# juanmc2005/diart

Measured on NVIDIA H100. Metric: audio-seconds/sec (real-time factor) at 5s/0.5s step, batch 256, higher is better.
Workload: dtype f32

## Files before the change

### diart_b200/csrc/api_seg.cu

```cuda
#include <math.h>
#include <string.h>

#include <algorithm>
#include <memory>
#include <vector>

#include "host.cuh"

namespace dg {

static void sinc_filters(const float* low_hz_, const float* band_hz_, std::vector<float>& filt ) {
  filt.assign(251 * 80, 0.f);
  float n_[125], win[125];
  for (int i = 0; i < 125; i++) {
    const float t = (float)(i - 125) / 16000.0f;
    n_[i] = 6.283185307179586f * t;
    win[i] = (float)(0.54 - 0.46 * cos(2.0 * M_PI * i / 250.0));
  }
  for (int f = 0; f < 40; f++) {
    const float low = 50.f + fabsf(low_hz_[f]);
    float high = low + 50.f + fabsf(band_hz_[f]);
    high = fminf(fmaxf(high, 50.f), 8000.f);
    const float band = high - low, two_band = 2.f * band;
    for (int i = 0; i < 125; i++) {
// ... 276 lines not shown
  h->K = (int)cn;
  const float* cw = t.get("classifier.weight", cn * 128);
  const float* cb = t.get("classifier.bias", cn);
  if (!cw || !cb) return DG_EWEIGHT;
  if (upload(h->cw, std::vector<float>(cw, cw + cn * 128)) || upload(h->cb, std::vector<float>(cb, cb + cn)))
    return DG_ECUDA;
  return 0;
}

extern "C" int dg_seg_create(const dg_tensor* tensors, int n, int device, dg_seg** out) {
  if (!tensors || !out) {
    set_error("dg_seg_create: null argument");
    return DG_EINVAL;
  }
  DG_CUDA(cudaSetDevice(device));
  std::unique_ptr<dg_seg> h(new dg_seg());
  h->device = device;
  Tensors t(tensors, n);
  int rc = seg_prepare(h.get(), t);
  if (rc) return rc;
  *out = h.release();
  return DG_OK;
}

extern "C" int dg_seg_dims(const dg_seg* h, int num_samples, int* frames, int* speakers) {
  if (!h || num_samples < 3000) {
    set_error("dg_seg_dims: bad arguments");
    return DG_EINVAL;
  }
  Geom g = make_geom(num_samples);
  if (frames) *frames = g.T2;
  if (speakers) *speakers = h->ps_speakers ? h->ps_speakers : h->K;
  return DG_OK;
}

extern "C" int dg_seg_set_powerset(dg_seg* h, int num_speakers, int max_per_frame) {
  if (!h || num_speakers < 1 || num_speakers > 8 || max_per_frame < 0 || max_per_frame > num_speakers) {
    set_error("dg_seg_set_powerset: bad arguments");
    return DG_EINVAL;
  }
  std::vector<uint32_t> masks;
  for (int size = 0; size <= max_per_frame; size++)
    for (uint32_t m = 0; m < (1u << num_speakers); m++) {
      if (__builtin_popcount(m) != size) continue;
      masks.push_back(m);
    }
  auto members = [&](uint32_t m) {
    std::vector<int> v;
    for (int i = 0; i < num_speakers; i++)
      if (m >> i & 1u) v.push_back(i);
    return v;
  };
  std::stable_sort(masks.begin(), masks.end(), [&](uint32_t a, uint32_t b) {
    const int sa = __builtin_popcount(a), sb = __builtin_popcount(b);
    if (sa != sb) return sa < sb;
    return members(a) < members(b);
  });
  if ((int)masks.size() != h->K) {
    set_error("dg_seg_set_powerset: the classifier has " + std::to_string(h->K) + " outputs but the powerset has " +
              std::to_string(masks.size()) + " classes");
    return DG_EINVAL;
  }
  DG_CUDA(cudaSetDevice(h->device));
  if (h->ps_masks.ensure(masks.size() * 4)) return DG_ECUDA;
  DG_CUDA(cudaMemcpy(h->ps_masks.p, masks.data(), masks.size() * 4, cudaMemcpyHostToDevice));
  h->ps_speakers = num_speakers;
  return DG_OK;
}

static int seg_head_final(dg_seg* h, const float* y2, int B, const Geom& g, float* seg, cudaStream_t st) {
  if (h->ps_speakers)
    return launch_seg_powerset(y2, h->cw.as<float>(), h->cb.as<float>(), B, g.T2, g.S2, h->K, h->ps_speakers,
                               h->ps_masks.as<unsigned>(), seg, st);
  return launch_seg_final(y2, h->cw.as<float>(), h->cb.as<float>(), B, g.T2, g.S2, h->K, seg, st);
}

int seg_forward_lane(dg_seg* h, int lane, const SincPrep* prep, const float* wav, int B, int S, float* seg,
                     cudaStream_t st, int stop_after) {
  DG_CUDA(cudaSetDevice(h->device));
  dg_seg::Scratch& w = h->scr[lane];
  const Geom g = make_geom(S);
  int rc;
  if ((rc = run_sincnet(h->sw, w.work, wav, B, g, st, prep))) return rc;
  const size_t rows = (size_t)B * g.S2 + 64;
  if (w.gx.ensure(rows * 1024 * 4) || w.y2.ensure(rows * 128 * 4) || w.xh.ensure(rows * 256 * 2) ||
      w.xl.ensure(rows * 256 * 2) || w.y1h.ensure(rows * 128 * 2) || w.y1l.ensure(rows * 128 * 2))
    return DG_ECUDA;
  const long long M = (long long)B * g.S2;
  if ((rc = launch_split_ex(w.work.out, M, 64, 64, 64, w.work.out_pool, g.S2, w.work.sc2.as<float>(), w.work.sh2.as<float>(),
                            w.xh.p, w.xl.p, st)))
    return rc;
  for (int L = 0; L < 4 && L <= stop_after; L++) {
    const int cin = L == 0 ? 64 : 256;
    TcGemm t{};
    t.A_hi = w.xh.p; t.A_lo = w.xl.p; t.lda = cin; t.Cin = cin; t.KW = 1; t.dil = 1; t.Mtot = M; t.M = M;
    t.N = 1024; t.bias = h->bih[L].as<float>(); t.out_f32 = w.gx.as<float>(); t.ldc = 1024; t.epi = 0; t.tag = "lstm_inproj";
    if ((rc = set_weights(t, h->wih[L])) || (rc = launch_gemm_tc(t, st))) return rc;
    if ((rc = launch_lstm_layer_tc(w.gx.as<float>(), h->whh[L].hi.p, h->whh[L].lo.p, h->whh[L].scale, B, g.T2, g.S2, nullptr,
                                   w.xh.p, w.xl.p, st)))
      return rc;
  }
  if (stop_after < 3) return 0;
  TcGemm t{};
  t.A_hi = w.xh.p; t.A_lo = w.xl.p; t.lda = 256; t.Cin = 256; t.KW = 1; t.dil = 1; t.Mtot = M; t.M = M;
  t.N = 128; t.bias = h->l1b.as<float>(); t.bn_scale = h->ones128.as<float>(); t.bn_shift = h->zeros128.as<float>();
  t.out_hi = w.y1h.p; t.out_lo = w.y1l.p; t.ldc = 128; t.epi = 1; t.tag = "seg_linear";
  if ((rc = set_weights(t, h->l1)) || (rc = launch_gemm_tc(t, st))) return rc;
  t.A_hi = w.y1h.p; t.A_lo = w.y1l.p; t.lda = 128; t.Cin = 128; t.bias = h->l2b.as<float>();
  t.out_hi = nullptr; t.out_lo = nullptr; t.out_f32 = w.y2.as<float>(); t.epi = 2;
  if ((rc = set_weights(t, h->l2)) || (rc = launch_gemm_tc(t, st))) return rc;
  return seg_head_final(h, w.y2.as<float>(), B, g, seg, st);
}

extern "C" int dg_seg_forward(dg_seg* h, const float* wav, int B, int S, float* seg, void* stream) {
  if (!h || !wav || !seg || B < 1 || S < 3000) {
    set_error("dg_seg_forward: bad arguments (need B >= 1, S >= 3000)");
    return DG_EINVAL;
  }
  cudaStream_t st = (cudaStream_t)stream;
  DG_CUDA(cudaSetDevice(h->device));
  LaneUse use(h->guard[0], stream ? stream : (void*)h, st);
  int rc;
  if ((rc = use.rc) || (rc = seg_forward_lane(h, 0, nullptr, wav, B, S, seg, st))) return rc;
  return use.end();
}

extern "C" int dg_seg_debug_stage(dg_seg* h, const float* wav_dev, int B, int S, int hop, int stage, float* out_host, int64_t cap,
                                  int* dims) {
  if (!h || !wav_dev || !out_host || !dims || B < 1 || S < 3000 || hop < 0 || stage < 0 || stage > 10 || h->ps_speakers) {
    set_error("dg_seg_debug_stage: bad arguments (need a multilabel segmentation handle, B >= 1, S >= 3000, stage 0..10)");
    return DG_EINVAL;
  }
  DG_CUDA(cudaSetDevice(h->device));
  const Geom g = make_geom(S);
  const char* who = "dg_seg_debug_stage";
  cudaStream_t st = nullptr;
  SincPrep shared;
  const SincPrep* prep = nullptr;
  DevBuf seg;
  int rc;
  if (seg.ensure((size_t)B * g.T2 * h->K * 4)) return DG_ECUDA;
  {
    LaneUse use(h->guard[0], h, st);
    if ((rc = use.rc)) return rc;
    if (hop > 0) {
      if ((rc = run_sinc_prep(shared, wav_dev, B, g, st, hop, false))) return rc;
      prep = &shared;
    }
    if ((rc = seg_forward_lane(h, 0, prep, wav_dev, B, S, seg.as<float>(), st, stage <= 3 ? -1 : stage <= 7 ? stage - 4 : 99)))
      return rc;
  }
  DG_CUDA(cudaDeviceSynchronize());
  if ((rc = debug_front_paths(prep, g, &dims[3]))) return rc;
  if (lstm_tc_rows(B) == 16) dims[3] |= DG_DBG_LSTM_16ROWS;
  const dg_seg::Scratch& w = h->scr[0];
  if (stage <= 3) return debug_copy_front(who, stage, w.work, prep, w.xh.p, w.xl.p, B, g, out_host, cap, dims);
  if (stage <= 7) return debug_copy_map(who, w.xh.p, w.xl.p, B, g.S2, 256, g.T2, 256, out_host, cap, dims);
  if (stage == 8) return debug_copy_map(who, w.y1h.p, w.y1l.p, B, g.S2, 128, g.T2, 128, out_host, cap, dims);
  if (stage == 9) return debug_copy_map(who, w.y2.p, nullptr, B, g.S2, 128, g.T2, 128, out_host, cap, dims);
  return debug_copy_map(who, seg.p, nullptr, B, g.T2, h->K, g.T2, h->K, out_host, cap, dims);
}

extern "C" int dg_seg_destroy(dg_seg* h) {
  delete h;
  return DG_OK;
}
```

### diart_b200/csrc/lstm_tc.cu

```cuda
#include <stdio.h>
#include <stdlib.h>
#include <string.h>

#include <vector>

#include "dg_common.cuh"
#include "tc_ptx.cuh"

namespace dg {

constexpr int LT_THREADS = 512;
constexpr int LT_WS_BYTES = 2 * 512 * 128;
__host__ __device__ constexpr int lt_plane(int nb) { return 128 * nb * 2; }
__host__ __device__ constexpr int lt_h_bytes(int nb) { return 2 * 2 * lt_plane(nb); }
__host__ __device__ constexpr int lt_x_bytes(int nb) { return 512 * nb * 4; }
constexpr int lt_smem(int nb) { return LT_WS_BYTES + lt_h_bytes(nb) + 2 * lt_x_bytes(nb) + 64 + 1024; }
static_assert(lt_smem(16) <= 227 * 1024, "lstm_tc: shared memory over the per-block limit");
static int lt_rows(int B) { return B >= 128 ? 16 : 8; }

__device__ __forceinline__ float ex2_approx(float x) {
  float y;
  asm("ex2.approx.ftz.f32 %0, %1;" : "=f"(y) : "f"(x));
  return y;
}
__device__ __forceinline__ float rcp_approx(float x) {
  float y;
  asm("rcp.approx.ftz.f32 %0, %1;" : "=f"(y) : "f"(x));
  return y;
}

__host__ __device__ constexpr int lt_row(int g, int u) { return (u >> 5) * 128 + (g >> 1) * 64 + ((u & 31) >> 3) * 16 + (g & 1) * 8 + (u & 7); }

template <int NB>
__global__ void __launch_bounds__(LT_THREADS, 1)
lstm_tc_kernel(const __grid_constant__ CUtensorMap tm_wlo, const __grid_constant__ CUtensorMap tm_gx,
               const uint16_t* __restrict__ w_hi , int B, int T, int stride, int groups_per_dir,
               float* __restrict__ hout, uint16_t* __restrict__ out_hi, uint16_t* __restrict__ out_lo, float acc_scale) {
  constexpr int LT_PLANE = lt_plane(NB), LT_H_BYTES = lt_h_bytes(NB), LT_X_BYTES = lt_x_bytes(NB);
  constexpr int E = NB / 4;
  extern __shared__ unsigned char smem_raw[];
  unsigned char* smem = reinterpret_cast<unsigned char*>((reinterpret_cast<uintptr_t>(smem_raw) + 1023) & ~uintptr_t(1023));
  unsigned char* wsm = smem;
  unsigned char* hsm = smem + LT_WS_BYTES;
  unsigned char* xsm = hsm + LT_H_BYTES;
  uint64_t* w_full = reinterpret_cast<uint64_t*>(xsm + 2 * LT_X_BYTES);
  uint64_t* x_full = w_full + 1;
  const int warp = threadIdx.x >> 5, lane = threadIdx.x & 31;
  const int wg = warp >> 2, wq = warp & 3;
  const int dir = blockIdx.x / groups_per_dir;
  const int b0 = (blockIdx.x - dir * groups_per_dir) * NB;
  const int t0 = dir == 0 ? 0 : T - 1;
  const int dt = dir == 0 ? 1 : -1;

  if (threadIdx.x == 0) {
    mbar_init(w_full, 1);
    mbar_init(&x_full[0], 1);
    mbar_init(&x_full[1], 1);
    asm volatile("fence.mbarrier_init.release.cluster;" ::: "memory");
  }
  for (int i = threadIdx.x; i < LT_H_BYTES / 4; i += LT_THREADS) reinterpret_cast<uint32_t*>(hsm)[i] = 0u;
  __syncthreads();
  if (threadIdx.x == 0) {
    mbar_expect_tx(w_full, LT_WS_BYTES);
    for (int kb = 0; kb < 2; kb++)
      for (int half = 0; half < 2; half++)
        tma_load_2d(wsm + kb * 65536 + half * 32768, &tm_wlo, kb * 64, dir * 512 + half * 256, w_full);
    mbar_expect_tx(&x_full[0], LT_X_BYTES);
    tma_load_4d(xsm, &tm_gx, 0, b0, dir * 16, t0, &x_full[0]);
  }
  uint32_t wa[2][8][4];
  {
    const uint32_t* src = reinterpret_cast<const uint32_t*>(w_hi + (size_t)dir * 512 * 128);
#pragma unroll
    for (int t = 0; t < 2; t++) {
      const int r0 = wg * 128 + t * 64 + wq * 16 + (lane >> 2);
#pragma unroll
      for (int ks = 0; ks < 8; ks++) {
        const int k2 = (ks * 16 + 2 * (lane & 3)) >> 1;
        wa[t][ks][0] = src[(size_t)r0 * 64 + k2];
        wa[t][ks][1] = src[(size_t)(r0 + 8) * 64 + k2];
        wa[t][ks][2] = src[(size_t)r0 * 64 + k2 + 4];
        wa[t][ks][3] = src[(size_t)(r0 + 8) * 64 + k2 + 4];
      }
    }
  }
  asm volatile("fence.proxy.async.shared::cta;" ::: "memory");
  __syncthreads();
  mbar_wait(w_full, 0);

  const int u = wg * 32 + wq * 8 + (lane >> 2);
  const int n0 = 2 * (lane & 3);
  auto ne = [](int e) { return (e & 1) + 8 * (e >> 1); };
  bool valid[E];
#pragma unroll
  for (int e = 0; e < E; e++) valid[e] = b0 + n0 + ne(e) < B;
  int hrow = (b0 + n0) * stride + t0;
  uint32_t x_addr[2];
#pragma unroll
  for (int j = 0; j < 2; j++) x_addr[j] = smem_u32(xsm) + wg * NB * 128 + (n0 + j) * 128 + ((((u & 31) >> 2) ^ (n0 + j)) << 4) + (u & 3) * 4;
  const uint32_t h_addr = smem_u32(hsm) + (u >> 3) * NB * 16 + n0 * 16 + (u & 7) * 2;
  const uint32_t wlo0 = smem_u32(wsm) + (wg * 128) * 128;
  const float L2E = 1.4426950408889634f;
  float c[E] = {};
  for (int step = 0; step < T; step++) {
    const int buf = step & 1;
    const uint32_t hb = smem_u32(hsm) + buf * (LT_H_BYTES / 2);
    uint32_t wlo = wlo0;
    asm volatile("" : "+r"(wlo));
    float acc[2][NB / 2];
    wg_fence();
#pragma unroll
    for (int ks = 0; ks < 8; ks++) {
      const uint64_t bh = wg_desc_plain(hb + ks * NB * 32, NB * 16, 128),
                     bl = wg_desc_plain(hb + LT_PLANE + ks * NB * 32, NB * 16, 128);
#pragma unroll
      for (int t = 0; t < 2; t++) {
        const uint64_t al = wg_desc(wlo + (ks >> 2) * 65536 + t * 64 * 128) + (uint64_t)(((ks & 3) * 32) >> 4);
        wgmma_rs<NB>(acc[t], wa[t][ks], bl, ks != 0);
        wgmma_ss<NB>(acc[t], al, bh, 1);
        wgmma_rs<NB>(acc[t], wa[t][ks], bh, 1);
      }
    }
    wg_commit();
    if (threadIdx.x == 0 && step + 1 < T) {
      uint64_t* bar = &x_full[(step + 1) & 1];
      mbar_expect_tx(bar, LT_X_BYTES);
      tma_load_4d(xsm + ((step + 1) & 1) * LT_X_BYTES, &tm_gx, 0, b0, dir * 16, t0 + (step + 1) * dt, bar);
    }
    wg_wait<0>();
    wg_fence_acc(acc[0]);
    wg_fence_acc(acc[1]);
    mbar_wait(&x_full[buf], (step >> 1) & 1);
    float h[E];
    uint16_t hh[E], hl[E];
#pragma unroll
    for (int e = 0; e < E; e++) {
      const int a = 4 * (e >> 1) + (e & 1);
      const uint32_t xa = x_addr[e & 1] + buf * LT_X_BYTES + (e >> 1) * 1024;
      float xg[4];
#pragma unroll
      for (int g = 0; g < 4; g++) asm volatile("ld.shared.f32 %0, [%1];" : "=f"(xg[g]) : "r"(xa + g * 4 * NB * 128) : "memory");
      const float di = 1.f + ex2_approx(fminf(fmaf(acc[0][a], acc_scale, xg[0]) * -L2E, 40.f));
      const float df = 1.f + ex2_approx(fminf(fmaf(acc[0][a + 2], acc_scale, xg[1]) * -L2E, 40.f));
      const float eg = ex2_approx(fminf(fmaf(acc[1][a], acc_scale, xg[2]) * (2.f * L2E), 40.f));
      const float p = di * (1.f + eg);
      c[e] = fmaf(c[e], p, (eg - 1.f) * df) * rcp_approx(p * df);
      const float ec = ex2_approx(fminf(c[e] * (2.f * L2E), 40.f));
      const float eo = ex2_approx(fminf(fmaf(acc[1][a + 2], acc_scale, xg[3]) * -L2E, 40.f));
      h[e] = valid[e] ? (ec - 1.f) * rcp_approx((1.f + eo) * (ec + 1.f)) : 0.f;
      split_h16(h[e], hh[e], hl[e]);
    }
    const uint32_t dst = h_addr + (buf ^ 1) * (LT_H_BYTES / 2);
#pragma unroll
    for (int e = 0; e < E; e++) {
      const uint32_t o = (e & 1) * 16 + (e >> 1) * 128;
      asm volatile("st.shared.u16 [%0], %1;" ::"r"(dst + o), "h"(hh[e]) : "memory");
      asm volatile("st.shared.u16 [%0], %1;" ::"r"(dst + LT_PLANE + o), "h"(hl[e]) : "memory");
    }
    asm volatile("fence.proxy.async.shared::cta;" ::: "memory");
    __syncthreads();
#pragma unroll
    for (int e = 0; e < E; e++)
      if (valid[e]) {
        const size_t o = (size_t)(hrow + ne(e) * stride) * 256 + dir * 128 + u;
        if (out_hi) {
          out_hi[o] = hh[e];
          out_lo[o] = hl[e];
        }
        if (hout) hout[o] = h[e];
      }
    hrow += dt;
  }
}

size_t lstm_tc_plane_elems() { return (size_t)2 * 512 * 128; }

float lstm_tc_pack_whh(const float* whh_fwd, const float* whh_bwd, uint16_t* hi, uint16_t* lo) {
  const float s0 = weight_plane_scale(whh_fwd, 512 * 128), s1 = weight_plane_scale(whh_bwd, 512 * 128);
  const float scale = s0 < s1 ? s0 : s1;
  std::vector<float> perm((size_t)512 * 128);
  for (int d = 0; d < 2; d++) {
    const float* w = d == 0 ? whh_fwd : whh_bwd;
    for (int g = 0; g < 4; g++)
      for (int u = 0; u < 128; u++) memcpy(&perm[(size_t)lt_row(g, u) * 128], w + ((size_t)g * 128 + u) * 128, 128 * sizeof(float));
    split_weights_host(perm.data(), 512, 512, 128, hi + (size_t)d * 512 * 128, lo + (size_t)d * 512 * 128, scale);
  }
  return scale;
}

int launch_lstm_layer_tc(const float* gx, const void* whh_hi, const void* whh_lo, float w_scale, int B, int T, int stride,
                         float* hout, void* out_hi, void* out_lo, cudaStream_t st) {
  ProfScope _ps("lstm_rec", st);
  EncodeTiledFn fn = encode_fn();
  if (!fn) {
    set_error("cuTensorMapEncodeTiled is not available from the driver");
    return -2;
  }
  if (!hout && !out_hi) {
    set_error("lstm_rec: no output buffer");
    return -1;
  }
  CUtensorMap tm;
  cuuint64_t dims[2] = {128, 1024};
  cuuint64_t strides[1] = {256};
  cuuint32_t box[2] = {64, 256};
  cuuint32_t estr[2] = {1, 1};
  if (fn(&tm, CU_TENSOR_MAP_DATA_TYPE_BFLOAT16, 2, const_cast<void*>(whh_lo), dims, strides, box, estr,
         CU_TENSOR_MAP_INTERLEAVE_NONE, CU_TENSOR_MAP_SWIZZLE_128B, CU_TENSOR_MAP_L2_PROMOTION_L2_256B,
         CU_TENSOR_MAP_FLOAT_OOB_FILL_NONE) != CUDA_SUCCESS) {
    set_error("cuTensorMapEncodeTiled failed for W_hh");
    return -2;
  }
  const int nb = lt_rows(B);
  CUtensorMap tmx;
  cuuint64_t xdims[4] = {32, (cuuint64_t)B, 32, (cuuint64_t)T};
  cuuint64_t xstrides[3] = {(cuuint64_t)stride * 4096, 128, 4096};
  cuuint32_t xbox[4] = {32, (cuuint32_t)nb, 16, 1};
  cuuint32_t xestr[4] = {1, 1, 1, 1};
  if (fn(&tmx, CU_TENSOR_MAP_DATA_TYPE_FLOAT32, 4, const_cast<float*>(gx), xdims, xstrides, xbox, xestr,
         CU_TENSOR_MAP_INTERLEAVE_NONE, CU_TENSOR_MAP_SWIZZLE_128B, CU_TENSOR_MAP_L2_PROMOTION_L2_256B,
         CU_TENSOR_MAP_FLOAT_OOB_FILL_NONE) != CUDA_SUCCESS) {
    set_error("cuTensorMapEncodeTiled failed for the LSTM gate rows");
    return -2;
  }
  auto kern = nb == 16 ? lstm_tc_kernel<16> : lstm_tc_kernel<8>;
  const int smem = lt_smem(nb);
  static bool attr_done[2][64] = {};
  if (first_use_on_device(attr_done[nb == 16])) DG_CUDA(cudaFuncSetAttribute(kern, cudaFuncAttributeMaxDynamicSharedMemorySize, smem));
  const int gpd = (B + nb - 1) / nb;
  const float inv = w_scale > 0.f ? 1.f / w_scale : 1.f;
  kern<<<2 * gpd, LT_THREADS, smem, st>>>(tm, tmx, reinterpret_cast<const uint16_t*>(whh_hi), B, T, stride, gpd, hout,
                                          reinterpret_cast<uint16_t*>(out_hi), reinterpret_cast<uint16_t*>(out_lo), inv);
  DG_LAUNCHED();
  return 0;
}

int lstm_tc_rows(int B) { return lt_rows(B); }
int lstm_tc_ctas(int B) { return 2 * ((B + lt_rows(B) - 1) / lt_rows(B)); }

}
```

### diart_b200/csrc/tc_ptx.cuh

```cuda
#pragma once
#include <cuda.h>
#include <cuda_bf16.h>
#include <stdint.h>

#include "dg_common.cuh"

namespace dg {

__device__ __forceinline__ uint32_t smem_u32(const void* p) { return (uint32_t)__cvta_generic_to_shared(p); }

__device__ __forceinline__ void mbar_init(uint64_t* bar, uint32_t count) {
  asm volatile("mbarrier.init.shared::cta.b64 [%0], %1;" ::"r"(smem_u32(bar)), "r"(count));
}
__device__ __forceinline__ void mbar_expect_tx(uint64_t* bar, uint32_t bytes) {
  asm volatile("mbarrier.arrive.expect_tx.shared::cta.b64 _, [%0], %1;" ::"r"(smem_u32(bar)), "r"(bytes) : "memory");
}
__device__ __forceinline__ void mbar_arrive(uint64_t* bar) {
  asm volatile("mbarrier.arrive.shared::cta.b64 _, [%0];" ::"r"(smem_u32(bar)) : "memory");
}
__device__ __forceinline__ bool mbar_try_wait(uint64_t* bar, uint32_t parity) {
  uint32_t ok;
  asm volatile(
      "{\n.reg .pred p;\nmbarrier.try_wait.parity.shared::cta.b64 p, [%1], %2;\nselp.u32 %0, 1, 0, p;\n}"
      : "=r"(ok)
      : "r"(smem_u32(bar)), "r"(parity)
      : "memory");
  return ok != 0;
}
__device__ __forceinline__ bool mbar_test_wait(uint64_t* bar, uint32_t parity) {
  uint32_t ok;
  asm volatile(
      "{\n.reg .pred p;\nmbarrier.test_wait.parity.shared::cta.b64 p, [%1], %2;\nselp.u32 %0, 1, 0, p;\n}"
      : "=r"(ok)
      : "r"(smem_u32(bar)), "r"(parity)
      : "memory");
  return ok != 0;
}
__device__ __forceinline__ void mbar_wait(uint64_t* bar, uint32_t parity) {
  if (mbar_try_wait(bar, parity)) return;
  const long long t0 = clock64();
  while (!mbar_try_wait(bar, parity)) {
    if (clock64() - t0 > 4000000000LL) __trap();
  }
}
__device__ __forceinline__ void tma_load_2d(void* smem_dst, const CUtensorMap* tmap, int c0, int c1, uint64_t* bar) {
  asm volatile(
      "cp.async.bulk.tensor.2d.shared::cluster.global.tile.mbarrier::complete_tx::bytes [%0], [%1, {%2, %3}], [%4];"
      ::"r"(smem_u32(smem_dst)), "l"(reinterpret_cast<uint64_t>(tmap)), "r"(c0), "r"(c1), "r"(smem_u32(bar))
      : "memory");
}
__device__ __forceinline__ void tma_load_4d(void* smem_dst, const CUtensorMap* tmap, int c0, int c1, int c2, int c3,
                                            uint64_t* bar) {
  asm volatile(
      "cp.async.bulk.tensor.4d.shared::cluster.global.tile.mbarrier::complete_tx::bytes [%0], [%1, {%2, %3, %4, %5}], [%6];"
      ::"r"(smem_u32(smem_dst)), "l"(reinterpret_cast<uint64_t>(tmap)), "r"(c0), "r"(c1), "r"(c2), "r"(c3), "r"(smem_u32(bar))
      : "memory");
}

__device__ __forceinline__ uint16_t f32_to_h16(float x) {
  uint16_t r;
  asm("cvt.rn.satfinite.f16.f32 %0, %1;" : "=h"(r) : "f"(x));
  return r;
}
__device__ __forceinline__ float h16_to_f32(uint16_t h) {
  float f;
  asm("cvt.f32.f16 %0, %1;" : "=f"(f) : "h"(h));
  return f;
}
__device__ __forceinline__ void split_h16(float x, uint16_t& hi, uint16_t& lo) {
  hi = f32_to_h16(x);
  lo = f32_to_h16(x - h16_to_f32(hi));
}
__device__ __forceinline__ uint32_t pack_u16x2(uint16_t a, uint16_t b) { return (uint32_t)a | ((uint32_t)b << 16); }

__device__ __forceinline__ void named_sync(int id, int n) { asm volatile("bar.sync %0, %1;" ::"r"(id), "r"(n) : "memory"); }
__device__ __forceinline__ void named_arrive(int id, int n) { asm volatile("bar.arrive %0, %1;" ::"r"(id), "r"(n) : "memory"); }
template <int R>
__device__ __forceinline__ void setmaxnreg_dec() { asm volatile("setmaxnreg.dec.sync.aligned.u32 %0;" ::"n"(R)); }
template <int R>
__device__ __forceinline__ void setmaxnreg_inc() { asm volatile("setmaxnreg.inc.sync.aligned.u32 %0;" ::"n"(R)); }

__device__ __forceinline__ void tma_store_2d(const CUtensorMap* tmap, const void* smem_src, int c0, int c1) {
  asm volatile("cp.async.bulk.tensor.2d.global.shared::cta.bulk_group [%0, {%2, %3}], [%1];"
               ::"l"(reinterpret_cast<uint64_t>(tmap)), "r"(smem_u32(smem_src)), "r"(c0), "r"(c1)
               : "memory");
}
__device__ __forceinline__ void fence_proxy_async_smem() { asm volatile("fence.proxy.async.shared::cta;" ::: "memory"); }
__device__ __forceinline__ void bulk_commit() { asm volatile("cp.async.bulk.commit_group;" ::: "memory"); }
__device__ __forceinline__ void bulk_wait_read_all() { asm volatile("cp.async.bulk.wait_group.read 0;" ::: "memory"); }
__device__ __forceinline__ void bulk_wait_all() { asm volatile("cp.async.bulk.wait_group 0;" ::: "memory"); }

__device__ __forceinline__ void st_shared_u32(uint32_t addr, uint32_t a) {
  asm volatile("st.shared.b32 [%0], %1;" ::"r"(addr), "r"(a) : "memory");
}
__device__ __forceinline__ void st_shared_v2(uint32_t addr, float a, float b) {
  asm volatile("st.shared.v2.f32 [%0], {%1, %2};" ::"r"(addr), "f"(a), "f"(b) : "memory");
}
__device__ __forceinline__ void st_shared_v4(uint32_t addr, uint32_t a, uint32_t b, uint32_t c, uint32_t d) {
  asm volatile("st.shared.v4.b32 [%0], {%1, %2, %3, %4};" ::"r"(addr), "r"(a), "r"(b), "r"(c), "r"(d) : "memory");
}


__device__ __forceinline__ uint64_t wg_desc(uint32_t smem_addr) {
  uint64_t d = 0;
  d |= (uint64_t)((smem_addr >> 4) & 0x3FFF);
  d |= (uint64_t)1 << 16;
  d |= (uint64_t)(1024 >> 4) << 32;
  d |= (uint64_t)1 << 62;
  return d;
}
__device__ __forceinline__ uint64_t wg_desc_sw64(uint32_t smem_addr) {
  uint64_t d = 0;
  d |= (uint64_t)((smem_addr >> 4) & 0x3FFF);
  d |= (uint64_t)1 << 16;
  d |= (uint64_t)(512 >> 4) << 32;
  d |= (uint64_t)2 << 62;
  return d;
}
__device__ __forceinline__ uint64_t wg_desc_plain(uint32_t smem_addr, uint32_t lbo, uint32_t sbo) {
  uint64_t d = 0;
  d |= (uint64_t)((smem_addr >> 4) & 0x3FFF);
  d |= (uint64_t)((lbo >> 4) & 0x3FFF) << 16;
  d |= (uint64_t)((sbo >> 4) & 0x3FFF) << 32;
  return d;
}
__device__ __forceinline__ void wg_fence() { asm volatile("wgmma.fence.sync.aligned;" ::: "memory"); }
__device__ __forceinline__ void wg_commit() { asm volatile("wgmma.commit_group.sync.aligned;" ::: "memory"); }
template <int N>
__device__ __forceinline__ void wg_wait() { asm volatile("wgmma.wait_group.sync.aligned %0;" ::"n"(N) : "memory"); }
template <int R>
__device__ __forceinline__ void wg_fence_acc(float (&d)[R]) {
#pragma unroll
  for (int i = 0; i < R; i++) asm volatile("" : "+f"(d[i])::"memory");
}

template <int N>
__device__ __forceinline__ void wgmma_ss(float (&d)[N / 2], uint64_t a, uint64_t b, uint32_t acc);
template <int N>
__device__ __forceinline__ void wgmma_rs(float (&d)[N / 2], const uint32_t (&a)[4], uint64_t b, uint32_t acc);

template <>
__device__ __forceinline__ void wgmma_ss<8>(float (&d)[4], uint64_t a, uint64_t b, uint32_t acc) {
  asm volatile("{\n.reg .pred p;\nsetp.ne.b32 p, %6, 0;\n"
               "wgmma.mma_async.sync.aligned.m64n8k16.f32.f16.f16 {%0, %1, %2, %3}, %4, %5, p, 1, 1, 0, 0;\n}"
               : "+f"(d[0]), "+f"(d[1]), "+f"(d[2]), "+f"(d[3])
               : "l"(a), "l"(b), "r"(acc));
}
template <>
__device__ __forceinline__ void wgmma_ss<16>(float (&d)[8], uint64_t a, uint64_t b, uint32_t acc) {
  asm volatile("{\n.reg .pred p;\nsetp.ne.b32 p, %10, 0;\n"
               "wgmma.mma_async.sync.aligned.m64n16k16.f32.f16.f16 {%0, %1, %2, %3, %4, %5, %6, %7}, %8, %9, p, 1, 1, 0, 0;\n}"
               : "+f"(d[0]), "+f"(d[1]), "+f"(d[2]), "+f"(d[3]), "+f"(d[4]), "+f"(d[5]), "+f"(d[6]), "+f"(d[7])
               : "l"(a), "l"(b), "r"(acc));
}
template <>
__device__ __forceinline__ void wgmma_ss<32>(float (&d)[16], uint64_t a, uint64_t b, uint32_t acc) {
  asm volatile("{\n.reg .pred p;\nsetp.ne.b32 p, %18, 0;\n"
               "wgmma.mma_async.sync.aligned.m64n32k16.f32.f16.f16 {%0, %1, %2, %3, %4, %5, %6, %7, %8, %9, %10, %11, %12, %13, %14, %15}, %16, %17, p, 1, 1, 0, 0;\n}"
               : "+f"(d[0]), "+f"(d[1]), "+f"(d[2]), "+f"(d[3]), "+f"(d[4]), "+f"(d[5]), "+f"(d[6]), "+f"(d[7]), "+f"(d[8]), "+f"(d[9]), "+f"(d[10]), "+f"(d[11]), "+f"(d[12]), "+f"(d[13]), "+f"(d[14]), "+f"(d[15])
               : "l"(a), "l"(b), "r"(acc));
}
template <>
__device__ __forceinline__ void wgmma_ss<64>(float (&d)[32], uint64_t a, uint64_t b, uint32_t acc) {
  asm volatile("{\n.reg .pred p;\nsetp.ne.b32 p, %34, 0;\n"
               "wgmma.mma_async.sync.aligned.m64n64k16.f32.f16.f16 {%0, %1, %2, %3, %4, %5, %6, %7, %8, %9, %10, %11, %12, %13, %14, %15, %16, %17, %18, %19, %20, %21, %22, %23, %24, %25, %26, %27, %28, %29, %30, %31}, %32, %33, p, 1, 1, 0, 0;\n}"
               : "+f"(d[0]), "+f"(d[1]), "+f"(d[2]), "+f"(d[3]), "+f"(d[4]), "+f"(d[5]), "+f"(d[6]), "+f"(d[7]), "+f"(d[8]), "+f"(d[9]), "+f"(d[10]), "+f"(d[11]), "+f"(d[12]), "+f"(d[13]), "+f"(d[14]), "+f"(d[15]), "+f"(d[16]), "+f"(d[17]), "+f"(d[18]), "+f"(d[19]), "+f"(d[20]), "+f"(d[21]), "+f"(d[22]), "+f"(d[23]), "+f"(d[24]), "+f"(d[25]), "+f"(d[26]), "+f"(d[27]), "+f"(d[28]), "+f"(d[29]), "+f"(d[30]), "+f"(d[31])
               : "l"(a), "l"(b), "r"(acc));
}
template <>
__device__ __forceinline__ void wgmma_ss<80>(float (&d)[40], uint64_t a, uint64_t b, uint32_t acc) {
  asm volatile("{\n.reg .pred p;\nsetp.ne.b32 p, %42, 0;\n"
               "wgmma.mma_async.sync.aligned.m64n80k16.f32.f16.f16 {%0, %1, %2, %3, %4, %5, %6, %7, %8, %9, %10, %11, %12, %13, %14, %15, %16, %17, %18, %19, %20, %21, %22, %23, %24, %25, %26, %27, %28, %29, %30, %31, %32, %33, %34, %35, %36, %37, %38, %39}, %40, %41, p, 1, 1, 0, 0;\n}"
               : "+f"(d[0]), "+f"(d[1]), "+f"(d[2]), "+f"(d[3]), "+f"(d[4]), "+f"(d[5]), "+f"(d[6]), "+f"(d[7]), "+f"(d[8]), "+f"(d[9]), "+f"(d[10]), "+f"(d[11]), "+f"(d[12]), "+f"(d[13]), "+f"(d[14]), "+f"(d[15]), "+f"(d[16]), "+f"(d[17]), "+f"(d[18]), "+f"(d[19]), "+f"(d[20]), "+f"(d[21]), "+f"(d[22]), "+f"(d[23]), "+f"(d[24]), "+f"(d[25]), "+f"(d[26]), "+f"(d[27]), "+f"(d[28]), "+f"(d[29]), "+f"(d[30]), "+f"(d[31]), "+f"(d[32]), "+f"(d[33]), "+f"(d[34]), "+f"(d[35]), "+f"(d[36]), "+f"(d[37]), "+f"(d[38]), "+f"(d[39])
               : "l"(a), "l"(b), "r"(acc));
}
template <>
__device__ __forceinline__ void wgmma_ss<128>(float (&d)[64], uint64_t a, uint64_t b, uint32_t acc) {
  asm volatile("{\n.reg .pred p;\nsetp.ne.b32 p, %66, 0;\n"
               "wgmma.mma_async.sync.aligned.m64n128k16.f32.f16.f16 {%0, %1, %2, %3, %4, %5, %6, %7, %8, %9, %10, %11, %12, %13, %14, %15, %16, %17, %18, %19, %20, %21, %22, %23, %24, %25, %26, %27, %28, %29, %30, %31, %32, %33, %34, %35, %36, %37, %38, %39, %40, %41, %42, %43, %44, %45, %46, %47, %48, %49, %50, %51, %52, %53, %54, %55, %56, %57, %58, %59, %60, %61, %62, %63}, %64, %65, p, 1, 1, 0, 0;\n}"
               : "+f"(d[0]), "+f"(d[1]), "+f"(d[2]), "+f"(d[3]), "+f"(d[4]), "+f"(d[5]), "+f"(d[6]), "+f"(d[7]), "+f"(d[8]), "+f"(d[9]), "+f"(d[10]), "+f"(d[11]), "+f"(d[12]), "+f"(d[13]), "+f"(d[14]), "+f"(d[15]), "+f"(d[16]), "+f"(d[17]), "+f"(d[18]), "+f"(d[19]), "+f"(d[20]), "+f"(d[21]), "+f"(d[22]), "+f"(d[23]), "+f"(d[24]), "+f"(d[25]), "+f"(d[26]), "+f"(d[27]), "+f"(d[28]), "+f"(d[29]), "+f"(d[30]), "+f"(d[31]), "+f"(d[32]), "+f"(d[33]), "+f"(d[34]), "+f"(d[35]), "+f"(d[36]), "+f"(d[37]), "+f"(d[38]), "+f"(d[39]), "+f"(d[40]), "+f"(d[41]), "+f"(d[42]), "+f"(d[43]), "+f"(d[44]), "+f"(d[45]), "+f"(d[46]), "+f"(d[47]), "+f"(d[48]), "+f"(d[49]), "+f"(d[50]), "+f"(d[51]), "+f"(d[52]), "+f"(d[53]), "+f"(d[54]), "+f"(d[55]), "+f"(d[56]), "+f"(d[57]), "+f"(d[58]), "+f"(d[59]), "+f"(d[60]), "+f"(d[61]), "+f"(d[62]), "+f"(d[63])
               : "l"(a), "l"(b), "r"(acc));
}
template <>
__device__ __forceinline__ void wgmma_rs<8>(float (&d)[4], const uint32_t (&a)[4], uint64_t b, uint32_t acc) {
  asm volatile("{\n.reg .pred p;\nsetp.ne.b32 p, %9, 0;\n"
               "wgmma.mma_async.sync.aligned.m64n8k16.f32.f16.f16 {%0, %1, %2, %3}, {%4, %5, %6, %7}, %8, p, 1, 1, 0;\n}"
               : "+f"(d[0]), "+f"(d[1]), "+f"(d[2]), "+f"(d[3])
               : "r"(a[0]), "r"(a[1]), "r"(a[2]), "r"(a[3]), "l"(b), "r"(acc));
}
template <>
__device__ __forceinline__ void wgmma_rs<16>(float (&d)[8], const uint32_t (&a)[4], uint64_t b, uint32_t acc) {
  asm volatile("{\n.reg .pred p;\nsetp.ne.b32 p, %13, 0;\n"
               "wgmma.mma_async.sync.aligned.m64n16k16.f32.f16.f16 {%0, %1, %2, %3, %4, %5, %6, %7}, {%8, %9, %10, %11}, %12, p, 1, 1, 0;\n}"
               : "+f"(d[0]), "+f"(d[1]), "+f"(d[2]), "+f"(d[3]), "+f"(d[4]), "+f"(d[5]), "+f"(d[6]), "+f"(d[7])
               : "r"(a[0]), "r"(a[1]), "r"(a[2]), "r"(a[3]), "l"(b), "r"(acc));
}

typedef CUresult (*EncodeTiledFn)(CUtensorMap*, CUtensorMapDataType, cuuint32_t, void*, const cuuint64_t*,
                                  const cuuint64_t*, const cuuint32_t*, const cuuint32_t*, CUtensorMapInterleave,
                                  CUtensorMapSwizzle, CUtensorMapL2promotion, CUtensorMapFloatOOBfill);

static inline EncodeTiledFn encode_fn() {
  static EncodeTiledFn fn = nullptr;
  if (!fn) {
    void* p = nullptr;
    cudaDriverEntryPointQueryResult q;
    if (cudaGetDriverEntryPoint("cuTensorMapEncodeTiled", &p, cudaEnableDefault, &q) == cudaSuccess &&
        q == cudaDriverEntryPointSuccess)
      fn = reinterpret_cast<EncodeTiledFn>(p);
  }
  return fn;
}

}
```

Measured before the change: 22870.

## Split LSTM recurrence across 2-CTA clusters with 32 rows and register-resident weights

For batches of 128 or more, the LSTM recurrence now runs on a new kernel that splits each direction's 512 gate rows across a pair of CTAs in a thread-block cluster. Each CTA keeps both the high and low halves of its W_hh share in registers and processes 32 batch rows per wgmma. Each step's hidden state is exchanged with the peer CTA through bulk DSMEM copies signalled by mbarriers. The aim is to cut per-step latency of the serial recurrence, since each CTA does half the gate work on a wider N. In exchange it adds cross-CTA synchronisation every timestep, higher register pressure, and the old 16-row path is removed.

Measured after the change: 23080 (median of 6 runs). No clear change (+0.9%).

```diff
diff --git a/diart_b200/csrc/api_seg.cu b/diart_b200/csrc/api_seg.cu
--- a/diart_b200/csrc/api_seg.cu
+++ b/diart_b200/csrc/api_seg.cu
@@ -452,7 +452,7 @@
   }
   DG_CUDA(cudaDeviceSynchronize());
   if ((rc = debug_front_paths(prep, g, &dims[3]))) return rc;
-  if (lstm_tc_rows(B) == 16) dims[3] |= DG_DBG_LSTM_16ROWS;
+  if (lstm_tc_rows(B) > 8) dims[3] |= DG_DBG_LSTM_16ROWS;
   const dg_seg::Scratch& w = h->scr[0];
   if (stage <= 3) return debug_copy_front(who, stage, w.work, prep, w.xh.p, w.xl.p, B, g, out_host, cap, dims);
   if (stage <= 7) return debug_copy_map(who, w.xh.p, w.xl.p, B, g.S2, 256, g.T2, 256, out_host, cap, dims);
diff --git a/diart_b200/csrc/lstm_tc.cu b/diart_b200/csrc/lstm_tc.cu
--- a/diart_b200/csrc/lstm_tc.cu
+++ b/diart_b200/csrc/lstm_tc.cu
@@ -15,8 +15,17 @@
 __host__ __device__ constexpr int lt_h_bytes(int nb) { return 2 * 2 * lt_plane(nb); }
 __host__ __device__ constexpr int lt_x_bytes(int nb) { return 512 * nb * 4; }
 constexpr int lt_smem(int nb) { return LT_WS_BYTES + lt_h_bytes(nb) + 2 * lt_x_bytes(nb) + 64 + 1024; }
-static_assert(lt_smem(16) <= 227 * 1024, "lstm_tc: shared memory over the per-block limit");
-static int lt_rows(int B) { return B >= 128 ? 16 : 8; }
+static_assert(lt_smem(8) <= 227 * 1024, "lstm_tc: shared memory over the per-block limit");
+constexpr int LC_ROWS = 32, LC_E = LC_ROWS / 4;
+constexpr int LC_THREADS = 256;
+constexpr int LC_PLANE = lt_plane(LC_ROWS);
+constexpr int LC_COPY = LC_PLANE / 4;
+constexpr int LC_BUF = 2 * LC_PLANE;
+constexpr int LC_H_BYTES = 2 * LC_BUF;
+constexpr int LC_X_BYTES = 256 * LC_ROWS * 4;
+constexpr int LC_SMEM = 2 * LC_X_BYTES + LC_H_BYTES + 64 + 1024;
+static_assert(LC_SMEM <= 227 * 1024, "lstm_tc: shared memory over the per-block limit");
+static int lt_rows(int B) { return B >= 128 ? LC_ROWS : 8; }
 
 __device__ __forceinline__ float ex2_approx(float x) {
   float y;
@@ -30,6 +39,19 @@
 }
 
 __host__ __device__ constexpr int lt_row(int g, int u) { return (u >> 5) * 128 + (g >> 1) * 64 + ((u & 31) >> 3) * 16 + (g & 1) * 8 + (u & 7); }
+
+__device__ __forceinline__ float lt_cell(float ai, float af, float ag, float ao, const float (&xg)[4], float acc_scale, float& c,
+                                         bool valid) {
+  const float L2E = 1.4426950408889634f;
+  const float di = 1.f + ex2_approx(fminf(fmaf(ai, acc_scale, xg[0]) * -L2E, 40.f));
+  const float df = 1.f + ex2_approx(fminf(fmaf(af, acc_scale, xg[1]) * -L2E, 40.f));
+  const float eg = ex2_approx(fminf(fmaf(ag, acc_scale, xg[2]) * (2.f * L2E), 40.f));
+  const float p = di * (1.f + eg);
+  c = fmaf(c, p, (eg - 1.f) * df) * rcp_approx(p * df);
+  const float ec = ex2_approx(fminf(c * (2.f * L2E), 40.f));
+  const float eo = ex2_approx(fminf(fmaf(ao, acc_scale, xg[3]) * -L2E, 40.f));
+  return valid ? (ec - 1.f) * rcp_approx((1.f + eo) * (ec + 1.f)) : 0.f;
+}
 
 template <int NB>
 __global__ void __launch_bounds__(LT_THREADS, 1)
@@ -100,7 +122,6 @@
   for (int j = 0; j < 2; j++) x_addr[j] = smem_u32(xsm) + wg * NB * 128 + (n0 + j) * 128 + ((((u & 31) >> 2) ^ (n0 + j)) << 4) + (u & 3) * 4;
   const uint32_t h_addr = smem_u32(hsm) + (u >> 3) * NB * 16 + n0 * 16 + (u & 7) * 2;
   const uint32_t wlo0 = smem_u32(wsm) + (wg * 128) * 128;
-  const float L2E = 1.4426950408889634f;
   float c[E] = {};
   for (int step = 0; step < T; step++) {
     const int buf = step & 1;
@@ -140,14 +161,7 @@
       float xg[4];
 #pragma unroll
       for (int g = 0; g < 4; g++) asm volatile("ld.shared.f32 %0, [%1];" : "=f"(xg[g]) : "r"(xa + g * 4 * NB * 128) : "memory");
-      const float di = 1.f + ex2_approx(fminf(fmaf(acc[0][a], acc_scale, xg[0]) * -L2E, 40.f));
-      const float df = 1.f + ex2_approx(fminf(fmaf(acc[0][a + 2], acc_scale, xg[1]) * -L2E, 40.f));
-      const float eg = ex2_approx(fminf(fmaf(acc[1][a], acc_scale, xg[2]) * (2.f * L2E), 40.f));
-      const float p = di * (1.f + eg);
-      c[e] = fmaf(c[e], p, (eg - 1.f) * df) * rcp_approx(p * df);
-      const float ec = ex2_approx(fminf(c[e] * (2.f * L2E), 40.f));
-      const float eo = ex2_approx(fminf(fmaf(acc[1][a + 2], acc_scale, xg[3]) * -L2E, 40.f));
-      h[e] = valid[e] ? (ec - 1.f) * rcp_approx((1.f + eo) * (ec + 1.f)) : 0.f;
+      h[e] = lt_cell(acc[0][a], acc[0][a + 2], acc[1][a], acc[1][a + 2], xg, acc_scale, c[e], valid[e]);
       split_h16(h[e], hh[e], hl[e]);
     }
     const uint32_t dst = h_addr + (buf ^ 1) * (LT_H_BYTES / 2);
@@ -171,6 +185,141 @@
       }
     hrow += dt;
   }
+}
+
+__global__ void __launch_bounds__(LC_THREADS, 1)
+lstm_tc_cluster_kernel(const __grid_constant__ CUtensorMap tm_gx, const uint16_t* __restrict__ w_hi, const uint16_t* __restrict__ w_lo,
+                       int B, int T, int stride, int groups_per_dir, float* __restrict__ hout, uint16_t* __restrict__ out_hi,
+                       uint16_t* __restrict__ out_lo, float acc_scale) {
+  extern __shared__ unsigned char smem_raw[];
+  unsigned char* smem = reinterpret_cast<unsigned char*>((reinterpret_cast<uintptr_t>(smem_raw) + 1023) & ~uintptr_t(1023));
+  unsigned char* xsm = smem;
+  unsigned char* hsm = xsm + 2 * LC_X_BYTES;
+  uint64_t* x_full = reinterpret_cast<uint64_t*>(hsm + LC_H_BYTES);
+  uint64_t* h_full = x_full + 2;
+  const uint32_t rank = cluster_ctarank(), peer = rank ^ 1;
+  const int warp = threadIdx.x >> 5, lane = threadIdx.x & 31;
+  const int wg = warp >> 2, wq = warp & 3;
+  const int gw = 2 * rank + wg;
+  const int cl = blockIdx.x >> 1;
+  const int dir = cl / groups_per_dir;
+  const int b0 = (cl - dir * groups_per_dir) * LC_ROWS;
+  const int t0 = dir == 0 ? 0 : T - 1;
+  const int dt = dir == 0 ? 1 : -1;
+
+  if (threadIdx.x == 0) {
+    for (int i = 0; i < 2; i++) {
+      mbar_init(&x_full[i], 1);
+      mbar_init(&h_full[i], 2);
+    }
+    asm volatile("fence.mbarrier_init.release.cluster;" ::: "memory");
+  }
+  for (int i = threadIdx.x; i < LC_H_BYTES / 4; i += LC_THREADS) reinterpret_cast<uint32_t*>(hsm)[i] = 0u;
+  asm volatile("fence.proxy.async.shared::cta;" ::: "memory");
+  cluster_sync();
+  auto load_x = [&](int step) {
+    uint64_t* bar = &x_full[step & 1];
+    mbar_expect_tx(bar, LC_X_BYTES);
+    tma_load_5d(xsm + (step & 1) * LC_X_BYTES, &tm_gx, 0, b0, 2 * rank, 4 * dir, t0 + step * dt, bar);
+  };
+  if (threadIdx.x == 0) load_x(0);
+  uint32_t wa[2][8][4], wl[2][8][4];
+  {
+    const uint32_t* src_hi = reinterpret_cast<const uint32_t*>(w_hi + (size_t)dir * 512 * 128);
+    const uint32_t* src_lo = reinterpret_cast<const uint32_t*>(w_lo + (size_t)dir * 512 * 128);
+#pragma unroll
+    for (int t = 0; t < 2; t++) {
+      const int r0 = gw * 128 + t * 64 + wq * 16 + (lane >> 2);
+#pragma unroll
+      for (int ks = 0; ks < 8; ks++) {
+        const int k2 = (ks * 16 + 2 * (lane & 3)) >> 1;
+        const size_t o[4] = {(size_t)r0 * 64 + k2, (size_t)(r0 + 8) * 64 + k2, (size_t)r0 * 64 + k2 + 4, (size_t)(r0 + 8) * 64 + k2 + 4};
+#pragma unroll
+        for (int i = 0; i < 4; i++) {
+          wa[t][ks][i] = src_hi[o[i]];
+          wl[t][ks][i] = src_lo[o[i]];
+        }
+      }
+    }
+  }
+
+  const int u = gw * 32 + wq * 8 + (lane >> 2);
+  const int n0 = 2 * (lane & 3);
+  auto ne = [](int e) { return (e & 1) + 8 * (e >> 1); };
+  uint32_t x_addr[2];
+#pragma unroll
+  for (int j = 0; j < 2; j++) x_addr[j] = smem_u32(xsm) + wg * LC_ROWS * 128 + (n0 + j) * 128 + ((((u & 31) >> 2) ^ (n0 + j)) << 4) + (u & 3) * 4;
+  const uint32_t h_addr = smem_u32(hsm) + (u >> 3) * LC_ROWS * 16 + n0 * 16 + (u & 7) * 2;
+  const uint32_t h_own = smem_u32(hsm) + gw * LC_COPY;
+  const uint32_t h_peer = cluster_map(h_own, peer), h_full_peer = cluster_map(smem_u32(h_full), peer);
+
+  float acc[2][LC_ROWS / 2], c[LC_E] = {};
+  for (int step = 0; step < T; step++) {
+    if (step > 0) mbar_wait(&h_full[step & 1], ((step - 1) >> 1) & 1);
+    const uint32_t hb = smem_u32(hsm) + (step & 1) * LC_BUF;
+    wg_fence();
+#pragma unroll
+    for (int ks = 0; ks < 8; ks++) {
+      const uint64_t bh = wg_desc_plain(hb + ks * LC_ROWS * 32, LC_ROWS * 16, 128),
+                     bl = wg_desc_plain(hb + LC_PLANE + ks * LC_ROWS * 32, LC_ROWS * 16, 128);
+#pragma unroll
+      for (int t = 0; t < 2; t++) {
+        wgmma_rs<LC_ROWS>(acc[t], wa[t][ks], bl, ks != 0);
+        wgmma_rs<LC_ROWS>(acc[t], wl[t][ks], bh, 1);
+        wgmma_rs<LC_ROWS>(acc[t], wa[t][ks], bh, 1);
+      }
+    }
+    wg_commit();
+    if (threadIdx.x == 0 && step + 1 < T) load_x(step + 1);
+    wg_wait<0>();
+    wg_fence_acc(acc[0]);
+    wg_fence_acc(acc[1]);
+    const int slot = step & 1;
+    mbar_wait(&x_full[slot], (step >> 1) & 1);
+    float h[LC_E];
+    uint16_t hh[LC_E], hl[LC_E];
+    const int rb = b0 + n0;
+#pragma unroll
+    for (int e = 0; e < LC_E; e++) {
+      const int a = 4 * (e >> 1) + (e & 1);
+      const uint32_t xa = x_addr[e & 1] + slot * LC_X_BYTES + (e >> 1) * 1024;
+      float xg[4];
+#pragma unroll
+      for (int g = 0; g < 4; g++) asm volatile("ld.shared.f32 %0, [%1];" : "=f"(xg[g]) : "r"(xa + g * 2 * LC_ROWS * 128) : "memory");
+      h[e] = lt_cell(acc[0][a], acc[0][a + 2], acc[1][a], acc[1][a + 2], xg, acc_scale, c[e], rb + ne(e) < B);
+      split_h16(h[e], hh[e], hl[e]);
+    }
+    if (step + 1 < T) {
+      const int nb = (step + 1) & 1;
+      const uint32_t dst = h_addr + nb * LC_BUF;
+#pragma unroll
+      for (int e = 0; e < LC_E; e++) {
+        const uint32_t o = (e & 1) * 16 + (e >> 1) * 128;
+        asm volatile("st.shared.u16 [%0], %1;" ::"r"(dst + o), "h"(hh[e]) : "memory");
+        asm volatile("st.shared.u16 [%0], %1;" ::"r"(dst + LC_PLANE + o), "h"(hl[e]) : "memory");
+      }
+      asm volatile("fence.proxy.async.shared::cta;" ::: "memory");
+      named_sync(1 + wg, 128);
+      if (threadIdx.x % 128 == 0) {
+        mbar_expect_tx(&h_full[nb], 2 * LC_COPY);
+        const uint32_t bar = h_full_peer + nb * 8;
+        bulk_copy_to_cluster(h_peer + nb * LC_BUF, h_own + nb * LC_BUF, LC_COPY, bar);
+        bulk_copy_to_cluster(h_peer + nb * LC_BUF + LC_PLANE, h_own + nb * LC_BUF + LC_PLANE, LC_COPY, bar);
+      }
+    }
+    const int frame = t0 + step * dt;
+#pragma unroll
+    for (int e = 0; e < LC_E; e++)
+      if (rb + ne(e) < B) {
+        const size_t o = ((size_t)(rb + ne(e)) * stride + frame) * 256 + dir * 128 + u;
+        if (out_hi) {
+          out_hi[o] = hh[e];
+          out_lo[o] = hl[e];
+        }
+        if (hout) hout[o] = h[e];
+      }
+  }
+  cluster_sync();
 }
 
 size_t lstm_tc_plane_elems() { return (size_t)2 * 512 * 128; }
@@ -199,6 +348,41 @@
   if (!hout && !out_hi) {
     set_error("lstm_rec: no output buffer");
     return -1;
+  }
+  const float inv = w_scale > 0.f ? 1.f / w_scale : 1.f;
+  if (lt_rows(B) == LC_ROWS) {
+    CUtensorMap tmx;
+    cuuint64_t xdims[5] = {32, (cuuint64_t)B, 4, 8, (cuuint64_t)T};
+    cuuint64_t xstrides[4] = {(cuuint64_t)stride * 4096, 128, 512, 4096};
+    cuuint32_t xbox[5] = {32, LC_ROWS, 2, 4, 1};
+    cuuint32_t xestr[5] = {1, 1, 1, 1, 1};
+    if (fn(&tmx, CU_TENSOR_MAP_DATA_TYPE_FLOAT32, 5, const_cast<float*>(gx), xdims, xstrides, xbox, xestr,
+           CU_TENSOR_MAP_INTERLEAVE_NONE, CU_TENSOR_MAP_SWIZZLE_128B, CU_TENSOR_MAP_L2_PROMOTION_L2_256B,
+           CU_TENSOR_MAP_FLOAT_OOB_FILL_NONE) != CUDA_SUCCESS) {
+      set_error("cuTensorMapEncodeTiled failed for the LSTM gate rows");
+      return -2;
+    }
+    static bool attr_done[64] = {};
+    if (first_use_on_device(attr_done))
+      DG_CUDA(cudaFuncSetAttribute(lstm_tc_cluster_kernel, cudaFuncAttributeMaxDynamicSharedMemorySize, LC_SMEM));
+    const int gpd = (B + LC_ROWS - 1) / LC_ROWS;
+    cudaLaunchConfig_t cfg = {};
+    cfg.gridDim = dim3(2 * 2 * gpd);
+    cfg.blockDim = dim3(LC_THREADS);
+    cfg.dynamicSmemBytes = LC_SMEM;
+    cfg.stream = st;
+    cudaLaunchAttribute attr[1];
+    attr[0].id = cudaLaunchAttributeClusterDimension;
+    attr[0].val.clusterDim.x = 2;
+    attr[0].val.clusterDim.y = 1;
+    attr[0].val.clusterDim.z = 1;
+    cfg.attrs = attr;
+    cfg.numAttrs = 1;
+    DG_CUDA(cudaLaunchKernelEx(&cfg, lstm_tc_cluster_kernel, tmx, reinterpret_cast<const uint16_t*>(whh_hi),
+                               reinterpret_cast<const uint16_t*>(whh_lo), B, T, stride, gpd, hout, reinterpret_cast<uint16_t*>(out_hi),
+                               reinterpret_cast<uint16_t*>(out_lo), inv));
+    DG_LAUNCHED();
+    return 0;
   }
   CUtensorMap tm;
   cuuint64_t dims[2] = {128, 1024};
@@ -211,7 +395,7 @@
     set_error("cuTensorMapEncodeTiled failed for W_hh");
     return -2;
   }
-  const int nb = lt_rows(B);
+  constexpr int nb = 8;
   CUtensorMap tmx;
   cuuint64_t xdims[4] = {32, (cuuint64_t)B, 32, (cuuint64_t)T};
   cuuint64_t xstrides[3] = {(cuuint64_t)stride * 4096, 128, 4096};
@@ -223,12 +407,11 @@
     set_error("cuTensorMapEncodeTiled failed for the LSTM gate rows");
     return -2;
   }
-  auto kern = nb == 16 ? lstm_tc_kernel<16> : lstm_tc_kernel<8>;
+  auto kern = lstm_tc_kernel<nb>;
   const int smem = lt_smem(nb);
-  static bool attr_done[2][64] = {};
-  if (first_use_on_device(attr_done[nb == 16])) DG_CUDA(cudaFuncSetAttribute(kern, cudaFuncAttributeMaxDynamicSharedMemorySize, smem));
+  static bool attr_done[64] = {};
+  if (first_use_on_device(attr_done)) DG_CUDA(cudaFuncSetAttribute(kern, cudaFuncAttributeMaxDynamicSharedMemorySize, smem));
   const int gpd = (B + nb - 1) / nb;
-  const float inv = w_scale > 0.f ? 1.f / w_scale : 1.f;
   kern<<<2 * gpd, LT_THREADS, smem, st>>>(tm, tmx, reinterpret_cast<const uint16_t*>(whh_hi), B, T, stride, gpd, hout,
                                           reinterpret_cast<uint16_t*>(out_hi), reinterpret_cast<uint16_t*>(out_lo), inv);
   DG_LAUNCHED();
@@ -236,6 +419,6 @@
 }
 
 int lstm_tc_rows(int B) { return lt_rows(B); }
-int lstm_tc_ctas(int B) { return 2 * ((B + lt_rows(B) - 1) / lt_rows(B)); }
-
-}
+int lstm_tc_ctas(int B) { return lt_rows(B) == LC_ROWS ? 2 * 2 * ((B + LC_ROWS - 1) / LC_ROWS) : 2 * ((B + 7) / 8); }
+
+}
diff --git a/diart_b200/csrc/tc_ptx.cuh b/diart_b200/csrc/tc_ptx.cuh
--- a/diart_b200/csrc/tc_ptx.cuh
+++ b/diart_b200/csrc/tc_ptx.cuh
@@ -55,6 +55,33 @@
       "cp.async.bulk.tensor.4d.shared::cluster.global.tile.mbarrier::complete_tx::bytes [%0], [%1, {%2, %3, %4, %5}], [%6];"
       ::"r"(smem_u32(smem_dst)), "l"(reinterpret_cast<uint64_t>(tmap)), "r"(c0), "r"(c1), "r"(c2), "r"(c3), "r"(smem_u32(bar))
       : "memory");
+}
+__device__ __forceinline__ void tma_load_5d(void* smem_dst, const CUtensorMap* tmap, int c0, int c1, int c2, int c3, int c4,
+                                            uint64_t* bar) {
+  asm volatile(
+      "cp.async.bulk.tensor.5d.shared::cluster.global.tile.mbarrier::complete_tx::bytes [%0], [%1, {%2, %3, %4, %5, %6}], [%7];"
+      ::"r"(smem_u32(smem_dst)), "l"(reinterpret_cast<uint64_t>(tmap)), "r"(c0), "r"(c1), "r"(c2), "r"(c3), "r"(c4),
+        "r"(smem_u32(bar))
+      : "memory");
+}
+
+__device__ __forceinline__ uint32_t cluster_ctarank() {
+  uint32_t r;
+  asm volatile("mov.u32 %0, %%cluster_ctarank;" : "=r"(r));
+  return r;
+}
+__device__ __forceinline__ uint32_t cluster_map(uint32_t smem_addr, uint32_t rank) {
+  uint32_t r;
+  asm volatile("mapa.shared::cluster.u32 %0, %1, %2;" : "=r"(r) : "r"(smem_addr), "r"(rank));
+  return r;
+}
+__device__ __forceinline__ void cluster_sync() {
+  asm volatile("barrier.cluster.arrive.release.aligned;\nbarrier.cluster.wait.acquire.aligned;" ::: "memory");
+}
+__device__ __forceinline__ void bulk_copy_to_cluster(uint32_t dst_cluster, uint32_t src, uint32_t bytes, uint32_t bar_cluster) {
+  asm volatile("cp.async.bulk.shared::cluster.shared::cta.mbarrier::complete_tx::bytes [%0], [%1], %2, [%3];"
+               ::"r"(dst_cluster), "r"(src), "r"(bytes), "r"(bar_cluster)
+               : "memory");
 }
 
 __device__ __forceinline__ uint16_t f32_to_h16(float x) {
@@ -193,6 +220,13 @@
   asm volatile("{\n.reg .pred p;\nsetp.ne.b32 p, %13, 0;\n"
                "wgmma.mma_async.sync.aligned.m64n16k16.f32.f16.f16 {%0, %1, %2, %3, %4, %5, %6, %7}, {%8, %9, %10, %11}, %12, p, 1, 1, 0;\n}"
                : "+f"(d[0]), "+f"(d[1]), "+f"(d[2]), "+f"(d[3]), "+f"(d[4]), "+f"(d[5]), "+f"(d[6]), "+f"(d[7])
+               : "r"(a[0]), "r"(a[1]), "r"(a[2]), "r"(a[3]), "l"(b), "r"(acc));
+}
+template <>
+__device__ __forceinline__ void wgmma_rs<32>(float (&d)[16], const uint32_t (&a)[4], uint64_t b, uint32_t acc) {
+  asm volatile("{\n.reg .pred p;\nsetp.ne.b32 p, %21, 0;\n"
+               "wgmma.mma_async.sync.aligned.m64n32k16.f32.f16.f16 {%0, %1, %2, %3, %4, %5, %6, %7, %8, %9, %10, %11, %12, %13, %14, %15}, {%16, %17, %18, %19}, %20, p, 1, 1, 0;\n}"
+               : "+f"(d[0]), "+f"(d[1]), "+f"(d[2]), "+f"(d[3]), "+f"(d[4]), "+f"(d[5]), "+f"(d[6]), "+f"(d[7]), "+f"(d[8]), "+f"(d[9]), "+f"(d[10]), "+f"(d[11]), "+f"(d[12]), "+f"(d[13]), "+f"(d[14]), "+f"(d[15])
                : "r"(a[0]), "r"(a[1]), "r"(a[2]), "r"(a[3]), "l"(b), "r"(acc));
 }
 
```
